# tberriel/OVO

Measured on AMD Instinct MI355X. Metric: frames/s (CLIP+SAM2+fusion+query), 640x480 ScanNet, 1/2/4/8 MI355X, higher is better.
Workload: dtype bf16; 1 GPU; BASELINE.json configs[2]: PE-Core-L14-336 TextRegion descriptors (2 x 336^2 crops of a 640x480 frame) + SAM2 hiera_b+ image encoder @1024^2 + back-projection + cull/project/match/vote on a 1000000-point map + multi-view fusion + dense per-point fusion + 10-prompt instance and dense-map query; every frame a keyframe; masks from the precomputed-mask seam (32/frame); map_points=1000000, texts=10, masks_per_frame=32, sam2=image encoder, masks=precomputed-mask seam (mask_generator.py:94-95), encoder_batch=14, dense_query=resident class map, rows touched by the keyframe re-evaluated, parallelism=single GPU, points_end=1366868, instances_end=242

## Files before the change

### include/ovo_hip.h

```cpp
#ifndef OVO_HIP_H
#define OVO_HIP_H

#include <stddef.h>
#include <stdint.h>

#ifdef __cplusplus
extern "C" {
#endif

#define OVO_OK 0
#define OVO_E_ARG (-1)
#define OVO_E_LAUNCH (-2)
#define OVO_E_UNSUPPORTED (-3)

typedef void *ovo_stream_t;

const char *ovo_hip_last_error(void);
int ovo_hip_abi_version(void);

int ovo_marker(int id, ovo_stream_t stream);
int ovo_profile_start(void);
int ovo_profile_stop(double *ms, double *work, int64_t *launches, int n_kinds);
int ovo_profile_bytes(double *bytes, int n_kinds);

// ... 144 lines not shown
int ovo_resize_normalize(const void *src, int src_dtype, int C, int H, int W, int y0, int x0, int ch, int cw,
                         float *out, int oh, int ow, int antialias, float scale, const float *mean3_host,
                         const float *std3_host, ovo_stream_t stream);

int ovo_resize_window_normalize(const void *src, int src_dtype, int C, int H, int W, int y0, int x0, int ch, int cw, float *out,
                                int oh, int ow, int virt_h, int virt_w, int top, int left, int filter, float scale,
                                const float *mean3_host, const float *std3_host, ovo_stream_t stream);
int ovo_resize_normalize_batch(const void *const *srcs_host, int n_src, int src_dtype, int C, int H, int W, const int32_t *crops_host, int n_crop,
                               float *out, int oh, int ow, int antialias, float scale, const float *mean3_host, const float *std3_host,
                               ovo_stream_t stream);

int ovo_mask_boxes(const uint8_t *masks, int n, int H, int W, int32_t *boxes_xywh, ovo_stream_t stream);
int ovo_mask_crops(const void *image, int img_dtype, int H, int W, const uint8_t *masks, const int32_t *boxes_xywh, int n,
                   int also_bbox, int margin, int R, int round_out, float *out, ovo_stream_t stream);

int ovo_rope_qk(void *qkv, int B, int T, int H, int hd, const float *cos_t, const float *sin_t, int t0,
                ovo_stream_t stream);

int ovo_feature_masks(const uint8_t *masks, int N, int H, int W, int gh, int gw, void *w, int gpad, float *cnt,
                      ovo_stream_t stream);

int ovo_stitch_tokens_t(const float *tokens, int tokens_per_crop, int t0, int d, int P, int nh, int nw, void *out,
                        int gpad, ovo_stream_t stream);

int ovo_unit_tokens(const void *x_t, int d, int G, int gpad, void *u_t, void *u, ovo_stream_t stream);
int ovo_global_patch_filter(const float *r_t, void *weights, int N, int G, int gpad, float th, float *cnt, ovo_stream_t stream);

int ovo_scale_rows_bf16(const float *x, const float *cnt, int N, int d, void *y, ovo_stream_t stream);
int ovo_l2_normalize_rows(const float *x, int64_t N, int d, float *y, ovo_stream_t stream);
int ovo_cast_f32(const float *x, int64_t n, void *y, int dtype, ovo_stream_t stream);

typedef struct {
    int32_t image_size, patch, width, layers, heads, mlp_dim, out_dim;
    int32_t n_prefix;
    int32_t act;
    int32_t pre_ln;
    int32_t use_rope;
    int32_t pool;
    int32_t kpad;
    float ln_eps;
    int32_t q_prescaled;
} ovo_vit_config_t;

typedef struct {
    const float *ln1_g, *ln1_b;
    const void *qkv_w; const float *qkv_b;
// ... 214 lines not shown
```

### ovo_amd/_lib.py

```python
from __future__ import annotations

import ctypes as C
import os
from typing import Optional

import torch

_HERE = os.path.dirname(os.path.abspath(__file__))
SO_PATH = os.path.join(_HERE, "lib", "libovo_hip.so")
ABI_VERSION = 19
E_UNSUPPORTED = -3


class OvoHipError(RuntimeError):
    pass


class Camera(C.Structure):
    _fields_ = [("aabb", C.c_float * 6), ("planes", C.c_float * 24), ("w2c", C.c_float * 16),
                ("K", C.c_float * 9), ("th", C.c_float), ("h", C.c_int32), ("w", C.c_int32)]


class Ratio(C.Structure):
    _fields_ = [("enabled", C.c_int32), ("r_h", C.c_float), ("r_w", C.c_float), ("crop_edge", C.c_int32)]
# ... 139 lines not shown
    "ovo_gemm_periodic": (_I32, [C.POINTER(Gemm), _I64, _P]),
    "ovo_gemm_unwindow": (_I32, [C.POINTER(Gemm), C.POINTER(Window), _P]),
    "ovo_gemm_fold_out": (_I32, [C.POINTER(Gemm), _P, _I64, _P, _I64, _P]),
    "ovo_gemm_fold_stats": (_I32, [_P, _I64, _I32, _I32, _P, _I64, _P, _P]),
    "ovo_gemm_fold_in": (_I32, [C.POINTER(Gemm), C.POINTER(Rope), _P, _I64, _I32, _I32, _P, _F32, _P]),
    "ovo_gemm_rowln": (_I32, [C.POINTER(Gemm), C.POINTER(Window), _P, _P, _F32, _P, _I64, _P]),
    "ovo_gemm_f32a": (_I32, [C.POINTER(Gemm), C.POINTER(Window), _P, C.c_int, _P, _P, C.c_float, C.c_int, C.c_int, _P]),
    "ovo_decode_best": (_I32, [_P, _I64, _F32, _P, _P, _P]),
    "ovo_attention": (_I32, [C.POINTER(Attention), _P]),
    "ovo_gemm_fewrows": (_I32, [C.POINTER(Gemm), _P]),
    "ovo_attention_short": (_I32, [_P, _I32, _I32, _I32, _I32, _F32, _P, _P]),
    "ovo_merge_clips": (_I32, [_P, _I64, _I32, _P, _I32, _I32, _P, _P]),
    "ovo_layernorm": (_I32, [_P, _I64, _I64, _I32, _P, _P, _F32, _P, _I64, _I32, _P]),
    "ovo_vit_embed": (_I32, [_P, _P, _I32, _P, _I32, _I32, _I32, _P, _P, _F32, _P, _P]),
    "ovo_im2col": (_I32, [_P, _I32, _I32, _I32, _I32, _I32, _I32, _I32, _P, _I32, _P]),
    "ovo_resize_normalize": (_I32, [_P, _I32, _I32, _I32, _I32, _I32, _I32, _I32, _I32, _P, _I32, _I32, _I32, _F32,
                                    C.POINTER(C.c_float), C.POINTER(C.c_float), _P]),
    "ovo_resize_normalize_batch": (_I32, [_P, _I32, _I32, _I32, _I32, _I32, _P, _I32, _P, _I32, _I32, _I32, _F32, _P, _P, _P]),
    "ovo_resize_window_normalize": (_I32, [_P, _I32, _I32, _I32, _I32, _I32, _I32, _I32, _I32, _P, _I32, _I32, _I32, _I32, _I32, _I32, _I32, _F32,
                                           C.POINTER(C.c_float), C.POINTER(C.c_float), _P]),
    "ovo_rope_qk": (_I32, [_P, _I32, _I32, _I32, _I32, _P, _P, _I32, _P]),
    "ovo_feature_masks": (_I32, [_P, _I32, _I32, _I32, _I32, _I32, _P, _I32, _P, _P]),
    "ovo_stitch_tokens_t": (_I32, [_P, _I32, _I32, _I32, _I32, _I32, _I32, _P, _I32, _P]),
    "ovo_unit_tokens": (_I32, [_P, _I32, _I32, _I32, _P, _P, _P]),
    "ovo_global_patch_filter": (_I32, [_P, _P, _I32, _I32, _I32, _F32, _P, _P]),
    "ovo_scale_rows_bf16": (_I32, [_P, _P, _I32, _I32, _P, _P]),
    "ovo_mlp_f32": (_I32, [_P, _I64, _I32, _P, _P, _F32, _P, _I64, _P, _I32, _P, _I64, _P, _P]),
    "ovo_neck_f32": (_I32, [_P, _I64, _I32, _P, _I64, _P, _I32, _P, _I64, _P, _P, _I32, _P]),
    "ovo_window_attention_f32": (_I32, [_P, _I32, _I32, _I32, _I32, _I32, _I32, _I32, _I32, _P, _P, _F32, _P, _I64, _P, _P, _I32, _P]),
    "ovo_l2_normalize_rows": (_I32, [_P, _I64, _I32, _P, _P]),
    "ovo_cast_f32": (_I32, [_P, _I64, _P, _I32, _P]),
    "ovo_row_epilogue": (_I32, [_P, _I64, _I32, _P, _I64, _P, _P, _F32, _P, _I64, _P, _P, _P, _P]),
    "ovo_sam_upscale_ln": (_I32, [_P, _P, _P, _P, _P, _F32, _I64, _I32, _I32, _P, _P]),
    "ovo_sam_upscale_masks": (_I32, [_P, _P, _P, _P, _I32, _I32, _I64, _I32, _I32, _P, _P]),
    "ovo_sam_linear": (_I32, [_P, _P, _P, _P, _I64, _I32, _P, _I32, _I64, _I32, _I32, _P]),
    "ovo_sam_proj_ln": (_I32, [_P, _P, _P, _P, _P, _I64, _P, _P, _F32, _P, _I64, _P, _P, _P, _I64, _I32, _I32, _P]),
    "ovo_sam_up1_ln": (_I32, [_P, _P, _P, _P, _P, _P, _F32, _I64, _I32, _I32, _I32, _P, _P]),
    "ovo_sam_up2_masks": (_I32, [_P, _P, _P, _P, _P, _I32, _I32, _I64, _I32, _I32, _I32, _P, _P]),
    "ovo_instance_moments": (_I32, [_P, _P, _I64, _I32, _P, _P, _P]),
    "ovo_near_fraction": (_I32, [_P, _P, _P, _I32, _I64, _F32, _P, _P]),
    "ovo_remap_instances": (_I32, [_P, _I64, _P, _I32, _P]),
    "ovo_map_reanchor_workspace_bytes": (_SZ, [_I32]),
    "ovo_map_reanchor": (_I32, [_P, _P, _P, _P, _I64, _P, _P, _P, _P, _I64, _P, _P, _P, _I32, _P, _SZ, _P]),
    "ovo_dense_repack_workspace_bytes": (_SZ, [_I32]),
    "ovo_dense_repack": (_I32, [_P, _P, _P, _P, _I32, _I32, _I64, _I64, _P, _P, _P, _P, _I64, _I32, _I32, _I32, _I64, _I64, _F32, _P, _P, _I32, _P, _SZ, _P]),
    "ovo_render_workspace_bytes": (_SZ, [_I32, _I32]),
# ... 196 lines not shown
```

### ovo_amd/build.py

```python
from __future__ import annotations

import concurrent.futures as cf
import os
import shutil
import subprocess
import sys

HERE = os.path.dirname(os.path.abspath(__file__))
CSRC = os.path.join(HERE, "csrc")
OUT_DIR = os.path.join(HERE, "lib")
OBJ_DIR = os.path.join(OUT_DIR, "obj")
SO = os.path.join(OUT_DIR, "libovo_hip.so")
ARCH = "gfx950"

COMMON = ["--offload-arch=" + ARCH, "-O3", "-std=c++17", "-fPIC", "-Wall", "-Wno-unused-function",
          "-Wno-unused-result", "-I" + os.path.join(os.path.dirname(HERE), "include")]
EXTRA = {"geometry.hip": ["-ffp-contract=off"], "render.hip": ["-ffp-contract=off"],
         "insgeo.hip": ["-ffp-contract=off"],
         "evalknn.hip": ["-ffp-contract=off"], "mlp_stream.hip": ["-fno-slp-vectorize"], "gemm_stream.hip": ["-fno-slp-vectorize"],
         "winattn.hip": ["-fno-slp-vectorize"], "gemm8p.hip": ["-fno-slp-vectorize"],
         "neck_stream.hip": ["-fno-slp-vectorize"],
         "merger.hip": ["-fno-slp-vectorize"]}


def hipcc() -> str:
    for c in (os.environ.get("HIPCC"), shutil.which("hipcc"), "/opt/rocm/bin/hipcc"):
        if c and os.path.exists(c):
            return c
    raise RuntimeError("hipcc not found: libovo_hip.so cannot be built")


def sources():
    return sorted(f for f in os.listdir(CSRC) if f.endswith(".hip"))


def _stale(target: str, deps) -> bool:
    if not os.path.exists(target):
        return True
    t = os.path.getmtime(target)
    return any(os.path.getmtime(d) > t for d in deps)


def _run(cmd, what: str) -> None:
    r = subprocess.run(cmd, capture_output=True, text=True)
    if r.returncode != 0:
# ... 45 lines not shown
```

### ovo_amd/csrc/encoder.hip

```cpp
#include <hip/hip_fp16.h>

#include "common.h"

namespace {

__device__ __forceinline__ float bf2f(uint16_t v) { return __uint_as_float((uint32_t)v << 16); }
__device__ __forceinline__ uint16_t f2bf(float x) {
    const __bf16 h = (__bf16)x;
    return *(const uint16_t *)&h;
}
__device__ __forceinline__ uint2 pack4_bf16(float a, float b, float c, float d) {
    return make_uint2((uint32_t)f2bf(a) | ((uint32_t)f2bf(b) << 16), (uint32_t)f2bf(c) | ((uint32_t)f2bf(d) << 16));
}

__device__ __forceinline__ void ln_row_wide(const float *__restrict__ x, int d, const float *__restrict__ gamma,
                                            const float *__restrict__ beta, float eps, void *__restrict__ y, int out_bf16, int lane,
                                            const float *__restrict__ extra_add) {
    const int d4 = d >> 2;
    float s = 0.f;
    for (int i = lane; i < d4; i += 64) {
        float4 v = ((const float4 *)x)[i];
        if (extra_add) { const float4 e = ((const float4 *)extra_add)[i]; v.x += e.x; v.y += e.y; v.z += e.z; v.w += e.w; }
        s += (v.x + v.y) + (v.z + v.w);
    }
// ... 429 lines not shown
        float v = 0.f;
        if (g < gh * gw) {
            const int gy = g / gw, gx = g % gw;
            float fy = sy * ((float)gy + 0.5f) - 0.5f; fy = fy < 0.f ? 0.f : fy;
            float fx = sx * ((float)gx + 0.5f) - 0.5f; fx = fx < 0.f ? 0.f : fx;
            const int y0 = (int)fy, x0 = (int)fx;
            const int y1 = y0 + (y0 < H - 1 ? 1 : 0), x1 = x0 + (x0 < W - 1 ? 1 : 0);
            const float ly = fy - (float)y0, lx = fx - (float)x0;
            const float a = m[(long long)y0 * W + x0] ? 1.f : 0.f, b = m[(long long)y0 * W + x1] ? 1.f : 0.f;
            const float c = m[(long long)y1 * W + x0] ? 1.f : 0.f, d = m[(long long)y1 * W + x1] ? 1.f : 0.f;
            v = (1.f - ly) * ((1.f - lx) * a + lx * b) + ly * ((1.f - lx) * c + lx * d);
        }
        const bool on = v > 0.f;
        w[(long long)n * gpad + g] = on ? 0x3f80 : 0;
        local += on;
    }
    __shared__ int red[256];
    red[threadIdx.x] = local;
    __syncthreads();
    for (int o = 128; o > 0; o >>= 1) { if (threadIdx.x < o) red[threadIdx.x] += red[threadIdx.x + o]; __syncthreads(); }
    if (threadIdx.x == 0) cnt[n] = (float)red[0];
}

__global__ void __launch_bounds__(256) k_stitch_t(const float *__restrict__ tokens, int tpc, int t0, int d, int P, int nh, int nw,
                                                  uint16_t *__restrict__ out, int gpad) {
    const int gh = P * nh, gw = P * nw, G = gh * gw;
    const long long total = (long long)d * gpad;
    const float sy = (float)P / (float)gh, sx = (float)P / (float)gw;
    for (long long i = (long long)blockIdx.x * blockDim.x + threadIdx.x; i < total; i += (long long)gridDim.x * blockDim.x) {
        const int g = (int)(i % gpad), c = (int)(i / gpad);
        float v = 0.f;
        if (g < G) {
            const int gy = g / gw, gx = g % gw;
            float fy = sy * ((float)gy + 0.5f) - 0.5f; fy = fy < 0.f ? 0.f : fy;
            float fx = sx * ((float)gx + 0.5f) - 0.5f; fx = fx < 0.f ? 0.f : fx;
            const int y0 = (int)fy, x0 = (int)fx;
            const int y1 = y0 + (y0 < P - 1 ? 1 : 0), x1 = x0 + (x0 < P - 1 ? 1 : 0);
            const float ly = fy - (float)y0, lx = fx - (float)x0;
            const float *glob = tokens + (long long)t0 * d + c;
            const float a = glob[(long long)(y0 * P + x0) * d], b = glob[(long long)(y0 * P + x1) * d];
            const float e = glob[(long long)(y1 * P + x0) * d], f = glob[(long long)(y1 * P + x1) * d];
            const float up = (1.f - ly) * ((1.f - lx) * a + lx * b) + ly * ((1.f - lx) * e + lx * f);
            const int tile = 1 + (gy / P) * nw + (gx / P);
            const float loc = tokens[((long long)tile * tpc + t0 + (gy % P) * P + (gx % P)) * d + c];
            v = 0.5f * up + loc;
        }
        out[i] = f2bf(v);
    }
}

__global__ void __launch_bounds__(256) k_unit_tokens(const uint16_t *__restrict__ x_t, int d, int G, int gpad, uint16_t *__restrict__ u_t,
                                                     uint16_t *__restrict__ u) {
    const int g = blockIdx.x * blockDim.x + threadIdx.x;
    if (g >= gpad) return;
    float ss = 0.f;
    if (g < G)
        for (int c = 0; c < d; ++c) { const float v = bf2f(x_t[(long long)c * gpad + g]); ss = fmaf(v, v, ss); }
    const float inv = g < G ? 1.0f / sqrtf(ss) : 0.f;
    for (int c = 0; c < d; ++c) {
        const uint16_t q = g < G ? f2bf(bf2f(x_t[(long long)c * gpad + g]) * inv) : (uint16_t)0;
        u_t[(long long)c * gpad + g] = q;
        u[(long long)g * d + c] = q;
    }
}

__global__ void __launch_bounds__(256) k_global_patch(const float *__restrict__ r_t, uint16_t *__restrict__ w, int N, int G, int gpad,
                                                      float th) {
    const int g = blockIdx.x * blockDim.x + threadIdx.x;
    if (g >= G) return;
    float belong = 0.f, outside = 0.f, nb = 0.f, no = 0.f;
    for (int n = 0; n < N; ++n) {
// ... 181 lines not shown
    return OVO_OK;
}

int ovo_feature_masks(const uint8_t *masks, int N, int H, int W, int gh, int gw, void *w, int gpad, float *cnt,
                      ovo_stream_t stream) {
    OVO_REQUIRE(N >= 0 && H > 0 && W > 0 && gh > 0 && gw > 0 && gpad >= gh * gw && gpad % 32 == 0, "bad shape");
    if (N == 0) return OVO_OK;
    OVO_REQUIRE(masks && w && cnt, "null pointer");
    k_feature_masks<<<N, 256, 0, (hipStream_t)stream>>>(masks, N, H, W, gh, gw, (uint16_t *)w, gpad, cnt);
    OVO_CHECK_LAUNCH();
    return OVO_OK;
}

int ovo_stitch_tokens_t(const float *tokens, int tokens_per_crop, int t0, int d, int P, int nh, int nw, void *out, int gpad,
                        ovo_stream_t stream) {
    OVO_REQUIRE(tokens && out && d > 0 && P > 0 && nh > 0 && nw > 0 && t0 >= 0, "bad argument");
    OVO_REQUIRE(tokens_per_crop >= t0 + P * P && gpad >= P * P * nh * nw && gpad % 32 == 0, "bad token / grid shape");
    k_stitch_t<<<ovo_grid((long long)d * gpad, 256), 256, 0, (hipStream_t)stream>>>(tokens, tokens_per_crop, t0, d, P, nh, nw,
                                                                                   (uint16_t *)out, gpad);
    OVO_CHECK_LAUNCH();
    return OVO_OK;
}

int ovo_unit_tokens(const void *x_t, int d, int G, int gpad, void *u_t, void *u, ovo_stream_t stream) {
    OVO_REQUIRE(x_t && u_t && u && d > 0 && G > 0 && gpad >= G, "bad argument");
    k_unit_tokens<<<(gpad + 255) / 256, 256, 0, (hipStream_t)stream>>>((const uint16_t *)x_t, d, G, gpad, (uint16_t *)u_t, (uint16_t *)u);
    OVO_CHECK_LAUNCH();
    return OVO_OK;
}

int ovo_global_patch_filter(const float *r_t, void *weights, int N, int G, int gpad, float th, float *cnt, ovo_stream_t stream) {
    OVO_REQUIRE(N >= 0 && G > 0 && gpad >= G, "bad shape");
    if (N == 0) return OVO_OK;
    OVO_REQUIRE(r_t && weights && cnt, "null pointer");
    k_global_patch<<<(G + 255) / 256, 256, 0, (hipStream_t)stream>>>(r_t, (uint16_t *)weights, N, G, gpad, th);
    k_row_count<<<N, 256, 0, (hipStream_t)stream>>>((const uint16_t *)weights, gpad, cnt);
    OVO_CHECK_LAUNCH();
    return OVO_OK;
}

int ovo_scale_rows_bf16(const float *x, const float *cnt, int N, int d, void *y, ovo_stream_t stream) {
    OVO_REQUIRE(N >= 0 && d > 0, "bad shape");
    if (N == 0) return OVO_OK;
    OVO_REQUIRE(x && cnt && y, "null pointer");
    k_scale_rows<<<ovo_grid((long long)N * d, 256), 256, 0, (hipStream_t)stream>>>(x, cnt, N, d, (uint16_t *)y);
    OVO_CHECK_LAUNCH();
// ... 23 lines not shown
```

### ovo_amd/entities/ovo.py

```python
from __future__ import annotations

import contextlib
import time
from collections import deque
from typing import Any, Dict, List, Optional, Tuple

import numpy as np
import torch

from .. import _lib as L
from ..utils import geometry_utils as G
from .descriptor_bank import DescriptorBank, KeyframeView
from .instance3d import Instance3D
from .token_lookahead import TokenLookahead


def _timed(slot: str):
    def deco(fn):
        def wrapper(self, *a, **k):
            if not self.config.get("log", False):
                return fn(self, *a, **k)
            torch.cuda.synchronize()
            t0 = time.time()
            out = fn(self, *a, **k)
# ... 452 lines not shown
        return self.lookahead

    def prefetch_image_features(self, image, image_ready=None) -> bool:
        la = self._lookahead()
        return la is not None and la.encode_one(image, image_ready)

    def prefetch_image_features_batch(self, images, ready=(), stream=None) -> bool:
        la = self._lookahead()
        return la is not None and la.encode(images, ready, stream)

    def discard_prefetched(self, image) -> None:
        if self.lookahead is not None:
            self.lookahead.discard(image)

    @_timed("t_clip")
    def _extract_clip(self, image: np.ndarray, binary_maps: torch.Tensor) -> torch.Tensor:
        if binary_maps is None:
            raise L.OvoHipError("_extract_clip: this keyframe's binary maps were not kept (track_finish(want_maps=False)): only its owner pools it")
        la = self.lookahead
        feats = la.take(image) if la is not None else None
        if feats is not None:
            tr = self.clip_generator.textregion
            tr._crops(*image.shape[:2])
            out = tr.pe_value_with_sam2_attn(tr.get_features_mask(binary_maps), feats) if binary_maps.shape[0] > 0 else \
                torch.empty((0, tr.out_dim), dtype=torch.float32, device=feats.device)
            la.release(image)
            return out
        if isinstance(image, torch.Tensor):
            img = image.to(self.bank.device).permute(2, 0, 1).contiguous()
        else:
            img = torch.from_numpy(np.ascontiguousarray(image.transpose((2, 0, 1)))).to(self.bank.device, non_blocking=True)
        with la.workspace() if la is not None else contextlib.nullcontext():
            return self.clip_generator.extract_clip(img, binary_maps, self.config.get("return_all_clips", False))

    @_timed("t_up")
    def _store_and_fuse(self, clip_embeds: torch.Tensor, matched_ins_ids: List[int], kf_id: int, updates) -> None:
        rows = self.bank.append(clip_embeds)
        self.keyframes["ins_descriptors"][kf_id] = KeyframeView(
            self.bank, {i: rows[j] for j, i in enumerate(matched_ins_ids) if i != -1})
        self._planned_kfs.discard(kf_id)
        desc = self.keyframes["ins_descriptors"]
        full = [(u[0], [desc[kf]._rows[u[0]] for kf in u[1]]) for u in updates if len(u) == 2]
        add = [(u[0], [desc[kf]._rows[u[0]] for kf in u[1]], u[2]) for u in updates if len(u) == 3]
        self.bank.fuse(full, Instance3D.mv_fusion)
        self.bank.fuse_add(add)

    def _update_matched_objects_clip(self, clip_embeds: torch.Tensor, matched_ins_ids: List[int], kf_id: int) -> None:
# ... 267 lines not shown
```

### ovo_amd/entities/textregion.py

```python
from __future__ import annotations

from typing import List, Optional, Tuple

import os

import numpy as np
import torch

from .. import _lib as L
from ..encoders.vit import HipViT


class PETextRegion(torch.nn.Module):
    def __init__(self, model: HipViT, model_card: str = "PE-Core-L14-336", preprocess=None,
                 resize_method: str = "multi_resolution", remove_global_patch: bool = True,
                 global_patch_threshold: float = 0.07, crop_size: Optional[int] = None, upsample_times: int = 1,
                 mask_type: str = "soft", dtype: str = "bf16", device=None, project_and_normalize: bool = True,
                 share_identical_crops: Optional[bool] = None):
        super().__init__()
        self.share_identical_crops = bool(int(os.environ.get("OVO_SHARE_CROPS", "0"))) if share_identical_crops is None else bool(share_identical_crops)
        self._uniq, self._crop_index = [0], [0]
        if not model_card.startswith("PE"):
            raise NotImplementedError("Current TextRegion implementaion supports only PE models.")
        self.remove_global_patch = bool(remove_global_patch)
# ... 50 lines not shown

    def forward_crops(self, h: int, w: int) -> List[Tuple[int, int, int, int]]:
        crops = self._crops(h, w)
        return [crops[k] for k in self._uniq]

    def get_img_features(self, image: torch.Tensor, scale: float = 1.0) -> torch.Tensor:
        _, h, w = image.shape
        batch = self.vlm.preprocess(image, self.forward_crops(h, w), scale=scale)
        return self.vlm.forward(batch, tokens=True)

    def get_features_mask(self, region_masks: torch.Tensor):
        m = region_masks.view(torch.uint8) if region_masks.dtype == torch.bool else \
            (region_masks if region_masks.dtype == torch.uint8 else region_masks.to(torch.uint8))
        m = L.dev(m.contiguous(), torch.uint8, "region_masks")
        n, h, w = m.shape
        g = self.points_per_h * self.points_per_w
        gpad = (g + 31) // 32 * 32
        weights = torch.empty((n, gpad), dtype=torch.bfloat16, device=m.device)
        cnt = torch.empty(n, dtype=torch.float32, device=m.device)
        L.check(L.load().ovo_feature_masks(L.ptr(m), n, h, w, self.points_per_h, self.points_per_w, L.ptr(weights), gpad,
                                           L.ptr(cnt), L.stream()))
        return weights, cnt

    def pe_value_with_sam2_attn(self, feature_masks, input_feature: torch.Tensor) -> torch.Tensor:
        weights, cnt = feature_masks
        tok = L.dev(input_feature, torch.float32, "input_feature")
        if tok.shape[0] == len(self._uniq) and len(self._uniq) != len(self._crop_index):
            tok = tok.index_select(0, torch.tensor(self._crop_index, dtype=torch.int64).to(tok.device, non_blocking=True))
        ncrop, tpc, d = tok.shape
        p = self.crop_size // self.patch_size
        t0 = 1 if self.vlm.spec.cls_token else 0
        nh, nw = (self.crop_num_h, self.crop_num_w) if self.resize_method == "multi_resolution" else (1, 1)
        if ncrop != 1 + nh * nw and self.resize_method == "multi_resolution":
            raise L.OvoHipError(f"expected {1 + nh * nw} crops, got {ncrop}")
        n, gpad = weights.shape
        lib = L.load()
        x_t = torch.empty((d, gpad), dtype=torch.bfloat16, device=tok.device)
        if self.resize_method == "multi_resolution":
            L.check(lib.ovo_stitch_tokens_t(L.ptr(tok), tpc, t0, d, p, nh, nw, L.ptr(x_t), gpad, L.stream()))
        else:
            x_t.zero_()
            x_t[:, :p * p] = tok[0, t0:].t().to(torch.bfloat16)
        if self.remove_global_patch and n > 0:
            weights, cnt = self._remove_global_patch(x_t, weights, cnt, nh * nw * p * p if self.resize_method == "multi_resolution" else p * p)
        sums = L.gemm(weights, x_t, torch.empty((n, d), dtype=torch.float32, device=tok.device))
        mean = torch.empty((n, d), dtype=torch.bfloat16, device=tok.device)
        L.check(lib.ovo_scale_rows_bf16(L.ptr(sums), L.ptr(cnt), n, d, L.ptr(mean), L.stream()))
        out = L.gemm(mean, self._fold_w, torch.empty((n, self.out_dim), dtype=torch.float32, device=tok.device), bias=self._fold_b)
        if not self.project_and_normalize:
            return out
        L.check(lib.ovo_l2_normalize_rows(L.ptr(out), n, self.out_dim, L.ptr(out), L.stream()))
        return out

    def _remove_global_patch(self, x_t: torch.Tensor, weights: torch.Tensor, cnt: torch.Tensor, g: int):
        lib = L.load()
        d, gpad = x_t.shape
        n = weights.shape[0]
        u_t = torch.empty_like(x_t)
        u = torch.empty((gpad, d), dtype=torch.bfloat16, device=x_t.device)
        L.check(lib.ovo_unit_tokens(L.ptr(x_t), d, g, gpad, L.ptr(u_t), L.ptr(u), L.stream()))
        sums = L.gemm(weights, u_t, torch.empty((n, d), dtype=torch.float32, device=x_t.device))
        mean = torch.empty((n, d), dtype=torch.bfloat16, device=x_t.device)
        L.check(lib.ovo_scale_rows_bf16(L.ptr(sums), L.ptr(cnt), n, d, L.ptr(mean), L.stream()))
        r_t = L.gemm(mean, u, torch.empty((n, gpad), dtype=torch.float32, device=x_t.device))
        weights, cnt = weights.clone(), torch.empty_like(cnt)
        L.check(lib.ovo_global_patch_filter(L.ptr(r_t), L.ptr(weights), n, g, gpad, self.global_patch_threshold, L.ptr(cnt), L.stream()))
        return weights, cnt

    def predict(self, image: torch.Tensor, region_masks: torch.Tensor, scale: float = 1.0) -> torch.Tensor:
        feats = self.get_img_features(image, scale=scale)
        return self.pe_value_with_sam2_attn(self.get_features_mask(region_masks), feats)
# ... 1 lines not shown
```

### ovo_amd/entities/token_lookahead.py

```python
from __future__ import annotations

import contextlib
import os
from typing import Dict

import torch

from .. import _lib as L
from ..utils.streams import side_stream


class TokenLookahead:
    def __init__(self, textregion, device) -> None:
        self.tr = textregion
        self.stream = side_stream(device, "OVO_VIT_CUS", int(os.environ.get("OVO_VIT_PRIORITY", "0")))
        self.widest = 0
        self._slots = [dict(batch=None, tokens=None, free=None, left=0) for _ in range(2)]
        self._next = 0
        self.reset()

    def reset(self) -> None:
        for slot in self._slots:
            slot["left"], slot["free"] = 0, None
        self._pending: Dict[int, tuple] = {}
        self._single = None
        self._newest = None
        self._outside = None
        self._last_read = None

    def idle(self) -> bool:
        return not self._pending and all(slot["left"] == 0 for slot in self._slots)

    def encode(self, images, ready=(), stream=None) -> bool:
        images = list(images)
        if not images or not all(isinstance(i, torch.Tensor) and i.is_cuda for i in images):
            return False
        slot = self._slots[self._next]
        if slot["left"] > 0:
            raise L.OvoHipError("TokenLookahead.encode: the batch before the previous one still has unconsumed images")
        self._next ^= 1
        tr, dev = self.tr, images[0].device
        h, w = images[0].shape[:2]
        crops = tr.forward_crops(h, w)
        nc, spec = len(crops), tr.vlm.spec
        n = len(images) * nc
        if slot["batch"] is None or slot["batch"].shape[0] < n:
            slot["batch"] = torch.empty((n, 3, spec.image_size, spec.image_size), dtype=torch.float32, device=dev)
            slot["tokens"] = torch.empty((n, spec.tokens, spec.width), dtype=torch.float32, device=dev)
        side = stream if stream is not None else self.stream
        for ev in (slot["free"], self._outside, *ready):
            if ev is not None:
                side.wait_event(ev)
        slot["free"] = self._outside = None
        with torch.cuda.stream(side):
            srcs = [image if image.dtype == torch.uint8 and image.is_contiguous() else image.permute(2, 0, 1).contiguous() for image in images]
            tr.vlm.preprocess_batch(srcs, crops, scale=1.0 / 255.0, out=slot["batch"][:n])
            tr.vlm.forward(slot["batch"][:n], tokens=True, out=slot["tokens"][:n])
            done = torch.cuda.Event()
            done.record(side)
        slot["left"] = len(images)
        self._newest = done
        self.widest = max(self.widest, len(images))
        for k, image in enumerate(images):
            self._pending[id(image)] = (image, slot["tokens"][k * nc:(k + 1) * nc], done, slot)
        return True

    def encode_one(self, image, ready=None) -> bool:
        if self._single is not None:
            self.discard(self._single)
        after = self._last_read
        if after is None:
            after = torch.cuda.Event()
            after.record()
        if not self.encode([image], [after, ready]):
            return False
        self._single = image
        return True

    def take(self, image):
        if self._single is not None and self._single is not image:
            self.discard(self._single)
        hit = self._pending.get(id(image))
        if hit is None or hit[0] is not image:
            return None
        torch.cuda.current_stream().wait_event(hit[2])
        return hit[1]

    def release(self, image) -> None:
        hit = self._drop(image)
        if hit is not None:
            slot = hit[3]
            slot["free"] = torch.cuda.Event()
            slot["free"].record()
            if slot["left"] == 0:
                self._last_read = slot["free"]

    def discard(self, image) -> None:
        hit = self._drop(image)
        if hit is not None and hit[3]["free"] is None:
            hit[3]["free"] = hit[2]

    def _drop(self, image):
        hit = self._pending.get(id(image))
        if hit is None or hit[0] is not image:
            return None
        del self._pending[id(image)]
        if image is self._single:
            self._single = None
        hit[3]["left"] -= 1
# ... 10 lines not shown
```

Before: 478.9 frames/s.

## Fuse region-descriptor pooling and batch token stitching on the side stream

Adds a fused region-descriptor path: one kernel resamples the masks onto the token grid, mask-pools the stitched tokens with MFMA and divides by the count. A second kernel applies the fold projection, adds the bias and L2-normalizes the rows using a ticket-based last-block reduction. This replaces the separate feature-mask, GEMM, scale, GEMM and normalize launches. Token stitching is also batched across frames and moved onto the lookahead encoder stream, so the main stream can reuse the precomputed x_t. The fused path covers only flags==0 and shapes under fixed limits and falls back otherwise, and the ticket scheme relies on careful fencing.

```diff
diff --git a/include/ovo_hip.h b/include/ovo_hip.h
--- a/include/ovo_hip.h
+++ b/include/ovo_hip.h
@@ -190,6 +190,13 @@
 
 int ovo_stitch_tokens_t(const float *tokens, int tokens_per_crop, int t0, int d, int P, int nh, int nw, void *out,
                         int gpad, ovo_stream_t stream);
+int ovo_stitch_tokens_t_batch(const float *tokens, int frames, int64_t frame_stride, int tokens_per_crop, int t0, int d, int P, int nh,
+                              int nw, void *out, int gpad, ovo_stream_t stream);
+
+size_t ovo_region_descriptors_workspace_bytes(int n, int d);
+int ovo_region_descriptors(const uint8_t *masks, int n, int H, int W, int gh, int gw, const void *x_t, int d, int gpad,
+                           const void *fold_w, const float *fold_b, int out_dim, int flags, float *out, void *ws, size_t ws_bytes,
+                           ovo_stream_t stream);
 
 int ovo_unit_tokens(const void *x_t, int d, int G, int gpad, void *u_t, void *u, ovo_stream_t stream);
 int ovo_global_patch_filter(const float *r_t, void *weights, int N, int G, int gpad, float th, float *cnt, ovo_stream_t stream);
diff --git a/ovo_amd/_lib.py b/ovo_amd/_lib.py
--- a/ovo_amd/_lib.py
+++ b/ovo_amd/_lib.py
@@ -185,6 +185,9 @@
     "ovo_rope_qk": (_I32, [_P, _I32, _I32, _I32, _I32, _P, _P, _I32, _P]),
     "ovo_feature_masks": (_I32, [_P, _I32, _I32, _I32, _I32, _I32, _P, _I32, _P, _P]),
     "ovo_stitch_tokens_t": (_I32, [_P, _I32, _I32, _I32, _I32, _I32, _I32, _P, _I32, _P]),
+    "ovo_stitch_tokens_t_batch": (_I32, [_P, _I32, _I64, _I32, _I32, _I32, _I32, _I32, _I32, _P, _I32, _P]),
+    "ovo_region_descriptors_workspace_bytes": (_SZ, [_I32, _I32]),
+    "ovo_region_descriptors": (_I32, [_P, _I32, _I32, _I32, _I32, _I32, _P, _I32, _I32, _P, _P, _I32, _I32, _P, _P, _SZ, _P]),
     "ovo_unit_tokens": (_I32, [_P, _I32, _I32, _I32, _P, _P, _P]),
     "ovo_global_patch_filter": (_I32, [_P, _P, _I32, _I32, _I32, _F32, _P, _P]),
     "ovo_scale_rows_bf16": (_I32, [_P, _P, _I32, _I32, _P, _P]),
diff --git a/ovo_amd/build.py b/ovo_amd/build.py
--- a/ovo_amd/build.py
+++ b/ovo_amd/build.py
@@ -20,7 +20,8 @@
          "evalknn.hip": ["-ffp-contract=off"], "mlp_stream.hip": ["-fno-slp-vectorize"], "gemm_stream.hip": ["-fno-slp-vectorize"],
          "winattn.hip": ["-fno-slp-vectorize"], "gemm8p.hip": ["-fno-slp-vectorize"],
          "neck_stream.hip": ["-fno-slp-vectorize"],
-         "merger.hip": ["-fno-slp-vectorize"]}
+         "merger.hip": ["-fno-slp-vectorize"],
+         "regiondesc.hip": ["-fno-slp-vectorize"]}
 
 
 def hipcc() -> str:
diff --git a/ovo_amd/csrc/encoder.hip b/ovo_amd/csrc/encoder.hip
--- a/ovo_amd/csrc/encoder.hip
+++ b/ovo_amd/csrc/encoder.hip
@@ -475,31 +475,45 @@
     if (threadIdx.x == 0) cnt[n] = (float)red[0];
 }
 
+__device__ __forceinline__ uint16_t stitch_element(const float *__restrict__ tokens, int tpc, int t0, int d, int P, int nw, int gw, int G, float sy, float sx,
+                                                   int g, int c) {
+    float v = 0.f;
+    if (g < G) {
+        const int gy = g / gw, gx = g % gw;
+        float fy = sy * ((float)gy + 0.5f) - 0.5f; fy = fy < 0.f ? 0.f : fy;
+        float fx = sx * ((float)gx + 0.5f) - 0.5f; fx = fx < 0.f ? 0.f : fx;
+        const int y0 = (int)fy, x0 = (int)fx;
+        const int y1 = y0 + (y0 < P - 1 ? 1 : 0), x1 = x0 + (x0 < P - 1 ? 1 : 0);
+        const float ly = fy - (float)y0, lx = fx - (float)x0;
+        const float *glob = tokens + (long long)t0 * d + c;
+        const float a = glob[(long long)(y0 * P + x0) * d], b = glob[(long long)(y0 * P + x1) * d];
+        const float e = glob[(long long)(y1 * P + x0) * d], f = glob[(long long)(y1 * P + x1) * d];
+        const float up = (1.f - ly) * ((1.f - lx) * a + lx * b) + ly * ((1.f - lx) * e + lx * f);
+        const int tile = 1 + (gy / P) * nw + (gx / P);
+        const float loc = tokens[((long long)tile * tpc + t0 + (gy % P) * P + (gx % P)) * d + c];
+        v = 0.5f * up + loc;
+    }
+    return f2bf(v);
+}
+
 __global__ void __launch_bounds__(256) k_stitch_t(const float *__restrict__ tokens, int tpc, int t0, int d, int P, int nh, int nw,
                                                   uint16_t *__restrict__ out, int gpad) {
     const int gh = P * nh, gw = P * nw, G = gh * gw;
     const long long total = (long long)d * gpad;
     const float sy = (float)P / (float)gh, sx = (float)P / (float)gw;
-    for (long long i = (long long)blockIdx.x * blockDim.x + threadIdx.x; i < total; i += (long long)gridDim.x * blockDim.x) {
-        const int g = (int)(i % gpad), c = (int)(i / gpad);
-        float v = 0.f;
-        if (g < G) {
-            const int gy = g / gw, gx = g % gw;
-            float fy = sy * ((float)gy + 0.5f) - 0.5f; fy = fy < 0.f ? 0.f : fy;
-            float fx = sx * ((float)gx + 0.5f) - 0.5f; fx = fx < 0.f ? 0.f : fx;
-            const int y0 = (int)fy, x0 = (int)fx;
-            const int y1 = y0 + (y0 < P - 1 ? 1 : 0), x1 = x0 + (x0 < P - 1 ? 1 : 0);
-            const float ly = fy - (float)y0, lx = fx - (float)x0;
-            const float *glob = tokens + (long long)t0 * d + c;
-            const float a = glob[(long long)(y0 * P + x0) * d], b = glob[(long long)(y0 * P + x1) * d];
-            const float e = glob[(long long)(y1 * P + x0) * d], f = glob[(long long)(y1 * P + x1) * d];
-            const float up = (1.f - ly) * ((1.f - lx) * a + lx * b) + ly * ((1.f - lx) * e + lx * f);
-            const int tile = 1 + (gy / P) * nw + (gx / P);
-            const float loc = tokens[((long long)tile * tpc + t0 + (gy % P) * P + (gx % P)) * d + c];
-            v = 0.5f * up + loc;
-        }
-        out[i] = f2bf(v);
-    }
+    for (long long i = (long long)blockIdx.x * blockDim.x + threadIdx.x; i < total; i += (long long)gridDim.x * blockDim.x)
+        out[i] = stitch_element(tokens, tpc, t0, d, P, nw, gw, G, sy, sx, (int)(i % gpad), (int)(i / gpad));
+}
+
+__global__ void __launch_bounds__(256) k_stitch_t_batch(const float *__restrict__ tokens, long long frame_stride, int tpc, int t0, int d, int P, int nh, int nw,
+                                                        uint16_t *__restrict__ out, int gpad) {
+    const int gh = P * nh, gw = P * nw, G = gh * gw;
+    const long long total = (long long)d * gpad;
+    const float sy = (float)P / (float)gh, sx = (float)P / (float)gw;
+    tokens += blockIdx.y * frame_stride;
+    out += blockIdx.y * total;
+    for (long long i = (long long)blockIdx.x * blockDim.x + threadIdx.x; i < total; i += (long long)gridDim.x * blockDim.x)
+        out[i] = stitch_element(tokens, tpc, t0, d, P, nw, gw, G, sy, sx, (int)(i % gpad), (int)(i / gpad));
 }
 
 __global__ void __launch_bounds__(256) k_unit_tokens(const uint16_t *__restrict__ x_t, int d, int G, int gpad, uint16_t *__restrict__ u_t,
@@ -727,6 +741,20 @@
     return OVO_OK;
 }
 
+int ovo_stitch_tokens_t_batch(const float *tokens, int frames, int64_t frame_stride, int tokens_per_crop, int t0, int d, int P, int nh, int nw, void *out,
+                              int gpad, ovo_stream_t stream) {
+    OVO_REQUIRE(frames >= 0 && frames <= 65535 && d > 0 && P > 0 && nh > 0 && nw > 0 && t0 >= 0, "bad argument");
+    OVO_REQUIRE(tokens_per_crop >= t0 + P * P && gpad >= P * P * nh * nw && gpad % 32 == 0, "bad token / grid shape");
+    OVO_REQUIRE(frame_stride >= (int64_t)(1 + nh * nw) * tokens_per_crop * d, "frame_stride is shorter than a frame's crops");
+    if (ovo_knob_set("OVO_REGION_DESC_SPLIT")) return OVO_E_UNSUPPORTED;
+    if (frames == 0) return OVO_OK;
+    OVO_REQUIRE(tokens && out, "null pointer");
+    k_stitch_t_batch<<<dim3(ovo_grid((long long)d * gpad, 256), frames), 256, 0, (hipStream_t)stream>>>(tokens, frame_stride, tokens_per_crop, t0, d, P, nh, nw,
+                                                                                                        (uint16_t *)out, gpad);
+    OVO_CHECK_LAUNCH();
+    return OVO_OK;
+}
+
 int ovo_unit_tokens(const void *x_t, int d, int G, int gpad, void *u_t, void *u, ovo_stream_t stream) {
     OVO_REQUIRE(x_t && u_t && u && d > 0 && G > 0 && gpad >= G, "bad argument");
     k_unit_tokens<<<(gpad + 255) / 256, 256, 0, (hipStream_t)stream>>>((const uint16_t *)x_t, d, G, gpad, (uint16_t *)u_t, (uint16_t *)u);
diff --git a/ovo_amd/csrc/regiondesc.hip b/ovo_amd/csrc/regiondesc.hip
--- /dev/null
+++ b/ovo_amd/csrc/regiondesc.hip
@@ -0,0 +1,184 @@
+#include "gemm_common.h"
+
+using ovo_gemm_detail::bf16x8;
+using ovo_gemm_detail::f32x4;
+using ovo_gemm_detail::Mfma;
+
+namespace {
+
+__device__ __forceinline__ uint16_t f2bf(float x) {
+    const __bf16 h = (__bf16)x;
+    return *(const uint16_t *)&h;
+}
+
+constexpr int RD_ROWS = 16;
+constexpr int RD_MR = 2;
+constexpr int RD_MAX_DIM = 1024;
+constexpr int RD_MAX_GPAD = 4096;
+constexpr int RD_MAX_ROWS = RD_ROWS * 4096;
+constexpr int RD_NT = 1024;
+constexpr int RD_KC = 6;
+
+__global__ void __launch_bounds__(RD_NT) k_region_mean(const uint8_t *__restrict__ masks, int N, int H, int W, int gh, int gw, const uint16_t *__restrict__ x_t,
+                                                     int d, int gpad, uint16_t *__restrict__ mean, unsigned int *__restrict__ ticket) {
+    extern __shared__ __attribute__((aligned(16))) char smem[];
+    const int ldw = gpad + 8;
+    uint16_t *w_s = (uint16_t *)smem;
+    int *cnt_s = (int *)(smem + (size_t)RD_MR * ldw * 2);
+    const int lane = threadIdx.x & 63, wave = threadIdx.x >> 6, fr = lane & 15, fq = lane >> 4;
+    const int row0 = blockIdx.y * RD_MR, ks_n = gpad / 32;
+    if (blockIdx.x == 0 && threadIdx.x == 0 && row0 % RD_ROWS == 0) ticket[row0 / RD_ROWS] = 0u;
+    if (threadIdx.x < RD_MR) cnt_s[threadIdx.x] = 0;
+    const int col0 = blockIdx.x * (RD_NT / 4) + wave * 16;
+    const bool cols = col0 < d;
+    const uint16_t *xa = x_t + (long long)(cols ? col0 + fr : 0) * gpad + fq * 8;
+    bf16x8 xf[2][RD_KC];
+    auto load_x = [&](bf16x8 (&f)[RD_KC], int c) {
+#pragma unroll
+        for (int k = 0; k < RD_KC; ++k)
+            if (cols && c * RD_KC + k < ks_n) f[k] = *(const bf16x8 *)(xa + (c * RD_KC + k) * 32);
+    };
+    load_x(xf[0], 0);
+    __syncthreads();
+    const float sy = (float)H / (float)gh, sx = (float)W / (float)gw;
+    const int G = gh * gw;
+    const uint8_t *tile_masks = masks + (long long)row0 * H * W;
+    for (int g = threadIdx.x; g < gpad; g += RD_NT) {
+        int y0 = 0, x0 = 0, y1 = 0, x1 = 0;
+        float ly = 0.f, lx = 0.f;
+        if (g < G) {
+            const int gy = g / gw, gx = g % gw;
+            float fy = sy * ((float)gy + 0.5f) - 0.5f; fy = fy < 0.f ? 0.f : fy;
+            float fx = sx * ((float)gx + 0.5f) - 0.5f; fx = fx < 0.f ? 0.f : fx;
+            y0 = (int)fy; x0 = (int)fx;
+            y1 = y0 + (y0 < H - 1 ? 1 : 0); x1 = x0 + (x0 < W - 1 ? 1 : 0);
+            ly = fy - (float)y0; lx = fx - (float)x0;
+        }
+        uint8_t a[RD_MR], b[RD_MR], c[RD_MR], e[RD_MR];
+#pragma unroll
+        for (int r = 0; r < RD_MR; ++r) {
+            a[r] = b[r] = c[r] = e[r] = 0;
+            if (g < G && row0 + r < N) {
+                const unsigned m = (unsigned)(r * H + y0) * W, m1 = (unsigned)(r * H + y1) * W;
+                a[r] = tile_masks[m + x0]; b[r] = tile_masks[m + x1];
+                c[r] = tile_masks[m1 + x0]; e[r] = tile_masks[m1 + x1];
+            }
+        }
+#pragma unroll
+        for (int r = 0; r < RD_MR; ++r) {
+            const float fa = a[r] ? 1.f : 0.f, fb = b[r] ? 1.f : 0.f, fc = c[r] ? 1.f : 0.f, fe = e[r] ? 1.f : 0.f;
+            const float v = (1.f - ly) * ((1.f - lx) * fa + lx * fb) + ly * ((1.f - lx) * fc + lx * fe);
+            const bool on = v > 0.f;
+            w_s[r * ldw + g] = on ? 0x3f80 : 0;
+            const unsigned long long set = __ballot(on);
+            if (lane == 0 && set) atomicAdd(&cnt_s[r], __popcll(set));
+        }
+    }
+    __syncthreads();
+    const uint16_t *wb = w_s + (fr < RD_MR ? fr : 0) * ldw + fq * 8;
+    f32x4 acc = {0.f, 0.f, 0.f, 0.f};
+    auto mma = [&](const bf16x8 (&f)[RD_KC], int c) {
+#pragma unroll
+        for (int k = 0; k < RD_KC; ++k)
+            if (c * RD_KC + k < ks_n) {
+                bf16x8 wfrag = *(const bf16x8 *)(wb + (c * RD_KC + k) * 32);
+                if (fr >= RD_MR) wfrag = bf16x8{0, 0, 0, 0, 0, 0, 0, 0};
+                acc = Mfma<bf16x8>::run(f[k], wfrag, acc);
+            }
+    };
+    if (!cols) return;
+    for (int c = 0; c * RD_KC < ks_n; c += 2) {
+        load_x(xf[1], c + 1);
+        mma(xf[0], c);
+        load_x(xf[0], c + 2);
+        mma(xf[1], c + 1);
+    }
+    if (fr < RD_MR && row0 + fr < N) {
+        const float cn = (float)cnt_s[fr];
+        uint2 p;
+        p.x = (uint32_t)f2bf(acc[0] / cn) | ((uint32_t)f2bf(acc[1] / cn) << 16);
+        p.y = (uint32_t)f2bf(acc[2] / cn) | ((uint32_t)f2bf(acc[3] / cn) << 16);
+        *(uint2 *)(mean + (long long)(row0 + fr) * d + col0 + fq * 4) = p;
+    }
+}
+
+constexpr int PJ_KS = RD_MAX_DIM / 32;
+__global__ void __launch_bounds__(256) k_region_project(const uint16_t *__restrict__ mean, int N, int d, const uint16_t *__restrict__ fold_w,
+                                                        const float *__restrict__ fold_b, int out, float *y, unsigned int *__restrict__ ticket) {
+    __shared__ int s_last;
+    const int lane = threadIdx.x & 63, wave = threadIdx.x >> 6, fr = lane & 15, fq = lane >> 4;
+    const int row0 = blockIdx.y * RD_ROWS, c0 = blockIdx.x * 64 + wave * 16, ks_n = d / 32;
+    const int mr = row0 + fr < N ? row0 + fr : N - 1;
+    const uint16_t *mp = mean + (long long)mr * d + fq * 8;
+    const uint16_t *wp = fold_w + (long long)(c0 + fr) * d + fq * 8;
+    const float4 b = *(const float4 *)(fold_b + c0 + fq * 4);
+    bf16x8 wf[PJ_KS], mf[PJ_KS];
+#pragma unroll
+    for (int k = 0; k < PJ_KS; ++k)
+        if (k < ks_n) { wf[k] = *(const bf16x8 *)(wp + k * 32); mf[k] = *(const bf16x8 *)(mp + k * 32); }
+    f32x4 acc = {0.f, 0.f, 0.f, 0.f};
+#pragma unroll
+    for (int k = 0; k < PJ_KS; ++k)
+        if (k < ks_n) acc = Mfma<bf16x8>::run(wf[k], mf[k], acc);
+    if (row0 + fr < N) *(float4 *)(y + (long long)(row0 + fr) * out + c0 + fq * 4) = make_float4(acc[0] + b.x, acc[1] + b.y, acc[2] + b.z, acc[3] + b.w);
+    __syncthreads();
+    if (threadIdx.x == 0) {
+        __threadfence();
+        s_last = atomicAdd(ticket + blockIdx.y, 1u) == gridDim.x - 1;
+    }
+    __syncthreads();
+    if (!s_last) return;
+    __threadfence();
+    constexpr int NV = RD_MAX_DIM / 64;
+    const int nv = out / 64;
+    float v[4][NV];
+#pragma unroll
+    for (int q = 0; q < 4; ++q) {
+        const int r = row0 + wave * 4 + q;
+#pragma unroll
+        for (int i = 0; i < NV; ++i)
+            if (i < nv && r < N) v[q][i] = y[(long long)r * out + lane + i * 64];
+    }
+#pragma unroll
+    for (int q = 0; q < 4; ++q) {
+        const int r = row0 + wave * 4 + q;
+        if (r >= N) break;
+        float s = 0.f;
+#pragma unroll
+        for (int i = 0; i < NV; ++i)
+            if (i < nv) s += v[q][i] * v[q][i];
+        const float inv = 1.0f / fmaxf(sqrtf(wave_sum(s)), 1e-12f);
+#pragma unroll
+        for (int i = 0; i < NV; ++i)
+            if (i < nv) y[(long long)r * out + lane + i * 64] = v[q][i] * inv;
+    }
+}
+
+bool rd_covers(int n, int H, int W, int d, int gpad, int out_dim, int flags) {
+    return flags == 0 && (long long)RD_MR * H * W < (1ll << 31) && n <= RD_MAX_ROWS && d <= RD_MAX_DIM && out_dim <= RD_MAX_DIM && d % 64 == 0 && out_dim % 64 == 0 && gpad <= RD_MAX_GPAD;
+}
+size_t rd_mean_bytes(int n, int d) { return ((size_t)n * d * 2 + 15) & ~(size_t)15; }
+
+}
+
+extern "C" size_t ovo_region_descriptors_workspace_bytes(int n, int d) {
+    if (n <= 0 || d <= 0) return 0;
+    return rd_mean_bytes(n, d) + (size_t)((n + RD_ROWS - 1) / RD_ROWS) * sizeof(unsigned int);
+}
+
+extern "C" int ovo_region_descriptors(const uint8_t *masks, int n, int H, int W, int gh, int gw, const void *x_t, int d, int gpad, const void *fold_w,
+                                      const float *fold_b, int out_dim, int flags, float *out, void *ws, size_t ws_bytes, ovo_stream_t stream) {
+    OVO_REQUIRE(n >= 0 && H > 0 && W > 0 && gh > 0 && gw > 0 && d > 0 && out_dim > 0 && gpad >= gh * gw && gpad % 32 == 0, "bad shape");
+    if (ovo_knob_set("OVO_REGION_DESC_SPLIT") || !rd_covers(n, H, W, d, gpad, out_dim, flags)) return OVO_E_UNSUPPORTED;
+    if (n == 0) return OVO_OK;
+    OVO_REQUIRE(masks && x_t && fold_w && fold_b && out && ws, "null pointer");
+    OVO_REQUIRE((((uintptr_t)x_t | (uintptr_t)fold_w | (uintptr_t)fold_b | (uintptr_t)out | (uintptr_t)ws) & 15) == 0, "operands must be 16-byte aligned");
+    OVO_REQUIRE(ws_bytes >= ovo_region_descriptors_workspace_bytes(n, d), "workspace too small (ovo_region_descriptors_workspace_bytes)");
+    const int tiles = (n + RD_ROWS - 1) / RD_ROWS;
+    const size_t lds = (size_t)RD_MR * (gpad + 8) * 2 + RD_MR * sizeof(int);
+    unsigned int *ticket = (unsigned int *)((char *)ws + rd_mean_bytes(n, d));
+    k_region_mean<<<dim3((d + RD_NT / 4 - 1) / (RD_NT / 4), (n + RD_MR - 1) / RD_MR), RD_NT, lds, (hipStream_t)stream>>>(masks, n, H, W, gh, gw, (const uint16_t *)x_t, d, gpad, (uint16_t *)ws, ticket);
+    k_region_project<<<dim3(out_dim / 64, tiles), 256, 0, (hipStream_t)stream>>>((const uint16_t *)ws, n, d, (const uint16_t *)fold_w, fold_b, out_dim, out, ticket);
+    OVO_CHECK_LAUNCH();
+    return OVO_OK;
+}
diff --git a/ovo_amd/entities/ovo.py b/ovo_amd/entities/ovo.py
--- a/ovo_amd/entities/ovo.py
+++ b/ovo_amd/entities/ovo.py
@@ -498,7 +498,7 @@
         if feats is not None:
             tr = self.clip_generator.textregion
             tr._crops(*image.shape[:2])
-            out = tr.pe_value_with_sam2_attn(tr.get_features_mask(binary_maps), feats) if binary_maps.shape[0] > 0 else \
+            out = tr.region_descriptors(binary_maps, feats, la.stitched(image)) if binary_maps.shape[0] > 0 else \
                 torch.empty((0, tr.out_dim), dtype=torch.float32, device=feats.device)
             la.release(image)
             return out
diff --git a/ovo_amd/entities/textregion.py b/ovo_amd/entities/textregion.py
--- a/ovo_amd/entities/textregion.py
+++ b/ovo_amd/entities/textregion.py
@@ -96,8 +96,7 @@
                                            L.ptr(cnt), L.stream()))
         return weights, cnt
 
-    def pe_value_with_sam2_attn(self, feature_masks, input_feature: torch.Tensor) -> torch.Tensor:
-        weights, cnt = feature_masks
+    def _stitch(self, input_feature: torch.Tensor, gpad: Optional[int] = None) -> torch.Tensor:
         tok = L.dev(input_feature, torch.float32, "input_feature")
         if tok.shape[0] == len(self._uniq) and len(self._uniq) != len(self._crop_index):
             tok = tok.index_select(0, torch.tensor(self._crop_index, dtype=torch.int64).to(tok.device, non_blocking=True))
@@ -107,20 +106,66 @@
         nh, nw = (self.crop_num_h, self.crop_num_w) if self.resize_method == "multi_resolution" else (1, 1)
         if ncrop != 1 + nh * nw and self.resize_method == "multi_resolution":
             raise L.OvoHipError(f"expected {1 + nh * nw} crops, got {ncrop}")
-        n, gpad = weights.shape
-        lib = L.load()
+        if gpad is None:
+            gpad = (self.points_per_h * self.points_per_w + 31) // 32 * 32
         x_t = torch.empty((d, gpad), dtype=torch.bfloat16, device=tok.device)
         if self.resize_method == "multi_resolution":
-            L.check(lib.ovo_stitch_tokens_t(L.ptr(tok), tpc, t0, d, p, nh, nw, L.ptr(x_t), gpad, L.stream()))
+            L.check(L.load().ovo_stitch_tokens_t(L.ptr(tok), tpc, t0, d, p, nh, nw, L.ptr(x_t), gpad, L.stream()))
         else:
             x_t.zero_()
             x_t[:, :p * p] = tok[0, t0:].t().to(torch.bfloat16)
+        return x_t
+
+    def stitch_batch(self, tokens: torch.Tensor, frames: int, out: torch.Tensor) -> bool:
+        if self.resize_method != "multi_resolution" or len(self._uniq) != len(self._crop_index):
+            return False
+        nc, (_, tpc, d) = len(self._crop_index), tokens.shape
+        rc = L.load().ovo_stitch_tokens_t_batch(L.ptr(L.dev(tokens, torch.float32, "tokens")), frames, nc * tpc * d, tpc, 1 if self.vlm.spec.cls_token else 0, d,
+                                                self.crop_size // self.patch_size, self.crop_num_h, self.crop_num_w,
+                                                L.ptr(L.dev(out, torch.bfloat16, "out")), out.shape[2], L.stream())
+        if rc != L.E_UNSUPPORTED:
+            L.check(rc)
+        return rc == 0
+
+    def region_descriptors(self, region_masks: torch.Tensor, input_feature: torch.Tensor, x_t: Optional[torch.Tensor] = None) -> torch.Tensor:
+        m = region_masks.view(torch.uint8) if region_masks.dtype == torch.bool else \
+            (region_masks if region_masks.dtype == torch.uint8 else region_masks.to(torch.uint8))
+        m = L.dev(m.contiguous(), torch.uint8, "region_masks")
+        n, h, w = m.shape
+        flags = (1 if self.remove_global_patch else 0) | (2 if self.resize_method != "multi_resolution" else 0) | (0 if self.project_and_normalize else 4)
+        if x_t is None:
+            x_t = self._stitch(input_feature)
+        d, gpad = x_t.shape
+        lib = L.load()
+        need = lib.ovo_region_descriptors_workspace_bytes(n, d)
+        ws = getattr(self, "_rd_ws", None)
+        if ws is None or ws.numel() < need or ws.device != m.device:
+            ws = self._rd_ws = torch.empty(max(need, 64 * d * 2), dtype=torch.uint8, device=m.device)
+        out = torch.empty((n, self.out_dim), dtype=torch.float32, device=m.device)
+        rc = lib.ovo_region_descriptors(L.ptr(m), n, h, w, self.points_per_h, self.points_per_w, L.ptr(x_t), d, gpad, L.ptr(self._fold_w), L.ptr(self._fold_b),
+                                        self.out_dim, flags, L.ptr(out), L.ptr(ws), ws.numel(), L.stream())
+        if rc == L.E_UNSUPPORTED:
+            return self._pool(self.get_features_mask(region_masks), x_t)
+        L.check(rc)
+        return out
+
+    def pe_value_with_sam2_attn(self, feature_masks, input_feature: torch.Tensor) -> torch.Tensor:
+        return self._pool(feature_masks, self._stitch(input_feature, feature_masks[0].shape[1]))
+
+    def _pool(self, feature_masks, x_t: torch.Tensor) -> torch.Tensor:
+        weights, cnt = feature_masks
+        lib = L.load()
+        (d, gpad), n, dev = x_t.shape, weights.shape[0], x_t.device
+        if gpad != weights.shape[1]:
+            raise L.OvoHipError(f"feature masks over {weights.shape[1]} grid columns, tokens over {gpad}")
+        p = self.crop_size // self.patch_size
+        nh, nw = (self.crop_num_h, self.crop_num_w) if self.resize_method == "multi_resolution" else (1, 1)
         if self.remove_global_patch and n > 0:
             weights, cnt = self._remove_global_patch(x_t, weights, cnt, nh * nw * p * p if self.resize_method == "multi_resolution" else p * p)
-        sums = L.gemm(weights, x_t, torch.empty((n, d), dtype=torch.float32, device=tok.device))
-        mean = torch.empty((n, d), dtype=torch.bfloat16, device=tok.device)
+        sums = L.gemm(weights, x_t, torch.empty((n, d), dtype=torch.float32, device=dev))
+        mean = torch.empty((n, d), dtype=torch.bfloat16, device=dev)
         L.check(lib.ovo_scale_rows_bf16(L.ptr(sums), L.ptr(cnt), n, d, L.ptr(mean), L.stream()))
-        out = L.gemm(mean, self._fold_w, torch.empty((n, self.out_dim), dtype=torch.float32, device=tok.device), bias=self._fold_b)
+        out = L.gemm(mean, self._fold_w, torch.empty((n, self.out_dim), dtype=torch.float32, device=dev), bias=self._fold_b)
         if not self.project_and_normalize:
             return out
         L.check(lib.ovo_l2_normalize_rows(L.ptr(out), n, self.out_dim, L.ptr(out), L.stream()))
diff --git a/ovo_amd/entities/token_lookahead.py b/ovo_amd/entities/token_lookahead.py
--- a/ovo_amd/entities/token_lookahead.py
+++ b/ovo_amd/entities/token_lookahead.py
@@ -15,7 +15,7 @@
         self.tr = textregion
         self.stream = side_stream(device, "OVO_VIT_CUS", int(os.environ.get("OVO_VIT_PRIORITY", "0")))
         self.widest = 0
-        self._slots = [dict(batch=None, tokens=None, free=None, left=0) for _ in range(2)]
+        self._slots = [dict(batch=None, tokens=None, x_t=None, free=None, left=0) for _ in range(2)]
         self._next = 0
         self.reset()
 
@@ -47,6 +47,9 @@
         if slot["batch"] is None or slot["batch"].shape[0] < n:
             slot["batch"] = torch.empty((n, 3, spec.image_size, spec.image_size), dtype=torch.float32, device=dev)
             slot["tokens"] = torch.empty((n, spec.tokens, spec.width), dtype=torch.float32, device=dev)
+        gpad = (tr.points_per_h * tr.points_per_w + 31) // 32 * 32
+        if slot["x_t"] is None or slot["x_t"].shape[0] < len(images) or tuple(slot["x_t"].shape[1:]) != (spec.width, gpad):
+            slot["x_t"] = torch.empty((len(images), spec.width, gpad), dtype=torch.bfloat16, device=dev)
         side = stream if stream is not None else self.stream
         for ev in (slot["free"], self._outside, *ready):
             if ev is not None:
@@ -56,13 +59,14 @@
             srcs = [image if image.dtype == torch.uint8 and image.is_contiguous() else image.permute(2, 0, 1).contiguous() for image in images]
             tr.vlm.preprocess_batch(srcs, crops, scale=1.0 / 255.0, out=slot["batch"][:n])
             tr.vlm.forward(slot["batch"][:n], tokens=True, out=slot["tokens"][:n])
+            stitched = tr.stitch_batch(slot["tokens"][:n], len(images), slot["x_t"])
             done = torch.cuda.Event()
             done.record(side)
         slot["left"] = len(images)
         self._newest = done
         self.widest = max(self.widest, len(images))
         for k, image in enumerate(images):
-            self._pending[id(image)] = (image, slot["tokens"][k * nc:(k + 1) * nc], done, slot)
+            self._pending[id(image)] = (image, slot["tokens"][k * nc:(k + 1) * nc], done, slot, slot["x_t"][k] if stitched else None)
         return True
 
     def encode_one(self, image, ready=None) -> bool:
@@ -85,6 +89,10 @@
             return None
         torch.cuda.current_stream().wait_event(hit[2])
         return hit[1]
+
+    def stitched(self, image):
+        hit = self._pending.get(id(image))
+        return hit[4] if hit is not None and hit[0] is image else None
 
     def release(self, image) -> None:
         hit = self._drop(image)
```

Measured after the change: 478.4 frames/s. About the same (-0.1%).
